# letitiabanana/PnP-OVSS

Measured on AMD Instinct MI355X. Metric: images/sec (336^2, drop_iter=4, blur+CRF), higher is better.
Workload: dtype bf16x3

## Files before the change

include/pnp_hip.h:

```cpp
#ifndef PNP_HIP_H
#define PNP_HIP_H

#include <stddef.h>
#include <stdint.h>

#ifdef __cplusplus
extern "C" {
#endif

typedef struct pnp_engine pnp_engine;

typedef struct pnp_config {
    int32_t img_size, patch, vit_dim, vit_depth, vit_heads, vit_mlp_ratio;
    float vit_ln_eps;
    int32_t txt_hidden, txt_layers, txt_heads, txt_inter;
    float txt_ln_eps;
    int32_t vocab, max_pos, enc_token_id;
    int32_t max_batch;
    int32_t max_text_len;
    int32_t stash_layer;
    int32_t compute_bf16;
    int32_t device;
} pnp_config;

// ... 226 lines not shown
enum { PNP_GEMM_G64 = 0, PNP_GEMM_G128 = 1, PNP_GEMM_G256 = 2, PNP_GEMM_WIDE = 3, PNP_GEMM_X3_WIDE = 4, PNP_GEMM_SMALL_X3 = 5 };
typedef struct pnp_gemm_plan {
    int32_t status;
    int32_t family;
    int32_t variant;
    int32_t dtype_bf16;
    int32_t n_pad;
    int32_t grid, block, smem;
    int32_t keeps_stamps;
    int32_t profiled;
    int32_t sk_full, sk_upw;
} pnp_gemm_plan;
int pnp_op_gemm_plan(int32_t form, int32_t M, int32_t N, int32_t K, int32_t lda, int32_t ldb, int32_t mode, int32_t has,
                     int32_t row_div, int32_t col_div, int32_t col_pad, int32_t n_cu, int32_t streamk_mode, int32_t sk_wgs,
                     pnp_gemm_plan* plan);
int pnp_op_vit_attention(int32_t bf16, const void* d_qk, int32_t ld_qk, int32_t D, const void* d_vt, int32_t ld_vt,
                         int32_t n_pad, void* d_ctx, int32_t B, int32_t heads, int32_t N, float scale, void* stream);
int pnp_op_vit_attention_x3(const void* d_qkv_hi, const void* d_qkv_lo, int32_t ld_qkv, int32_t D, void* d_ctx_hi, void* d_ctx_lo,
                            int32_t B, int32_t heads, int32_t N, float scale, void* stream);
int pnp_op_layernorm(const float* d_x, const float* d_w, const float* d_b, float eps, int32_t rows, int32_t D,
                     float* d_y, void* stream);
int pnp_op_xattn(int32_t bf16, int32_t mode, const void* d_nat, int32_t ld_nat, const void* d_tr, int32_t ld_tr,
                 int32_t n_pad, const void* d_x, int32_t ldx, void* d_out, int32_t ldo, float* d_probs, int32_t n_stride,
                 int32_t B, int32_t L, int32_t N, int32_t heads, void* stream);
int pnp_dbg_gemm_stamps(uint64_t* host_out, int32_t max_blocks);
int pnp_op_cast(int32_t to_bf16, const float* d_in, void* d_out, int64_t n, void* stream);
int pnp_op_sort_pairs(uint64_t* d_keys_in, uint64_t* d_keys_out, uint32_t* d_vals_in, uint32_t* d_vals_out, int64_t n,
                      int32_t begin_bit, int32_t end_bit, const size_t* h_seg_off, int32_t n_seg, void* stream);
int pnp_op_scan_i32(const int32_t* d_in, int32_t* d_out, int64_t n, int32_t inclusive, void* stream);
int pnp_op_text_self_attn(int32_t bf16, const void* d_qkv, const int64_t* d_mask, int32_t ld_mask, void* d_ctx, float* d_probs,
// ... 21 lines not shown
```

pnp-ovss_amd/csrc/kernels.h:

```cpp
#pragma once
#include <hip/hip_runtime.h>
#include <stdint.h>
#include <stddef.h>
#include "gemm.h"

namespace pnp {

struct PostDesc {
    int H, W, K, C, has_bg, pix0;
    int Kp;
    int G, Kg;
    size_t off;
    size_t qoff;
    size_t voff[2];
};

struct alignas(16) CrfEntry {
    uint32_t pixel;
    float w;
    float nr;
    uint32_t pad;
};

struct alignas(16) CrfNbr8 {
// ... 53 lines not shown

int gradcam_gather(const float* P, const float* dP, const int64_t* mask, int ld_mask, float* out, int B, int nheads,
                   int head, int L, int Nst, int PP, hipStream_t s);
int drop_step(const float* G, float* g0, float* agg, uint8_t* dropped, int32_t* picks, int iter, int B, int T, int PP,
              int npick, int max_picks, hipStream_t s);
int merge_tokens(const float* src, const int32_t* cls_off, const int32_t* tok_idx, const int32_t* cls_div,
                 const int32_t* img_cls_off, float* out, int B, int T, int PP, int Cmax, hipStream_t s);
int threshold_maps(const float* merged, const int32_t* img_cls_off, float* out, float threshold, int B, int PP, int Cmax,
                   hipStream_t s);
int upsample_maps(const float* src, const PostDesc* desc, float* maps, int B, int P, int Cmax, int maxHW, hipStream_t s);
int minmax_normalize(float* maps, const PostDesc* desc, float* stats, int B, int Kmax, int maxHW, int class_channels_only,
                     hipStream_t s);
int background_channel(float* maps, const PostDesc* desc, int B, int maxHW, hipStream_t s);
int blur_maps(const float* in, float* tmp, float* out, const PostDesc* desc, const double* wts, const int32_t* wt_off,
              int B, int Kmax, int maxH, int maxW, int max_radius, hipStream_t s);
int preprocess_images(const uint8_t* rgb, const void* desc, int B, int S, int max_H, const int32_t* coef, uint8_t* tmp,
                      const float* mean3, const float* std3, float* out, hipStream_t s);
int unary_from_maps(const float* maps, const PostDesc* desc, float* unary, int B, int maxHW, int max_kp, int group, hipStream_t s);
int argmax_remap(const float* q, const PostDesc* desc, const int32_t* lut, int lut_stride, uint8_t* labels,
                 const size_t* label_off, int pixel_major, int group, int B, int maxHW, hipStream_t s);
int confusion_hist(const uint8_t* labels, const float* gt, const PostDesc* desc, const size_t* label_off,
                   unsigned long long* hist, int n_class, int B, int maxHW, hipStream_t s);

struct JpegImage {
    int64_t data_off;
    int64_t coef_off[3];
    int64_t plane_off[3];
    int64_t rgb_off;
    int32_t data_len, H, W, ncomp, hmax, vmax, mcux, mcuy;
    int32_t h[3], v[3], tq[3], td[3], ta[3], bx[3], by[3];
// ... 74 lines not shown
```

pnp-ovss_amd/csrc/ops.hip:

```cpp
#include <cstring>

#include "engine.h"

using namespace pnp;

extern "C" int pnp_itc_similarity(const float* d_img_feat, const float* d_txt_feat, int32_t B, int32_t T, int32_t E, float* d_sim,
                                  void* stream) {
    if (!d_img_feat || !d_txt_feat || !d_sim || B <= 0 || T <= 0 || E <= 0 || E % 4) return PNP_ERR_ARG;
    return itc_similarity(d_img_feat, d_txt_feat, d_sim, B, T, E, (hipStream_t)stream);
}

static GemmArgs gemm_op_args(const void* A, const void* A_lo, int lda, const void* B, const void* B_lo, int ldb, int M, int N, int K,
                             const float* bias, int bias_on_rows, const float* resid, int ldr, float* out_f32, int ldo, void* out_t,
                             void* out_lo, int ldo_t, int mode, float* aux, int ld_aux, int row_div, int col_div, int col_pad) {
    GemmArgs g = G_(A, lda, B, ldb, M, N, K);
    g.A_lo = A_lo; g.B_lo = B_lo;
    g.bias = bias; g.bias_on_rows = bias_on_rows; g.resid = resid; g.ldr = ldr;
    g.out_f32 = out_f32; g.ldo = ldo; g.out_t = out_t; g.out_lo = out_lo; g.ldo_t = ldo_t;
    g.mode = mode; g.aux = aux; g.ld_aux = ld_aux; g.row_div = row_div; g.col_div = col_div; g.col_pad = col_pad;
    return g;
}

extern "C" int pnp_op_gemm_ex(int32_t bf, const void* d_A, int32_t lda, const void* d_B, int32_t ldb, int32_t M, int32_t N,
                              int32_t K, const float* d_bias, const float* d_resid, int32_t ldr, float* d_out_f32, int32_t ldo,
// ... 86 lines not shown
extern "C" int pnp_op_gemm_plan(int32_t form, int32_t M, int32_t N, int32_t K, int32_t lda, int32_t ldb, int32_t mode, int32_t has,
                                int32_t row_div, int32_t col_div, int32_t col_pad, int32_t n_cu, int32_t streamk_mode, int32_t sk_wgs,
                                pnp_gemm_plan* plan) {
    if (!plan || form < PNP_GEMM_FORM_F32 || form > PNP_GEMM_FORM_X3A) return PNP_ERR_ARG;
    static float there[4];
    auto p = [&](int bit) { return (has & bit) ? there : nullptr; };
    const bool x3 = form == PNP_GEMM_FORM_X3, x3a = form == PNP_GEMM_FORM_X3A;
    GemmArgs g = gemm_op_args(there, x3 ? there : nullptr, lda, there, x3 || x3a ? there : nullptr, ldb, M, N, K, p(PNP_GEMM_HAS_BIAS),
                              (has & PNP_GEMM_HAS_BIAS_ON_ROWS) ? 1 : 0, p(PNP_GEMM_HAS_RESID), 0, p(PNP_GEMM_HAS_OUT_F32), 0, p(PNP_GEMM_HAS_OUT_T),
                              p(PNP_GEMM_HAS_OUT_LO), 0, mode, p(PNP_GEMM_HAS_AUX), 0, row_div, col_div, col_pad);
    g.a_f32 = x3a;
    *plan = gemm_plan(form == PNP_GEMM_FORM_BF16 || x3, g, n_cu, streamk_mode, sk_wgs);
    return plan->status;
}

extern "C" int pnp_op_vit_attention(int32_t bf, const void* d_qk, int32_t ld_qk, int32_t D, const void* d_vt, int32_t ld_vt,
                                    int32_t n_pad, void* d_ctx, int32_t B, int32_t heads, int32_t N, float scale, void* stream) {
    if (!d_qk || !d_vt || !d_ctx || B <= 0 || heads <= 0 || N <= 0) return PNP_ERR_ARG;
    return vit_attention(bf, d_qk, ld_qk, D, d_vt, ld_vt, n_pad, d_ctx, B, heads, N, scale, (hipStream_t)stream);
}

extern "C" int pnp_op_vit_attention_x3(const void* d_qkv_hi, const void* d_qkv_lo, int32_t ld_qkv, int32_t D, void* d_ctx_hi,
                                       void* d_ctx_lo, int32_t B, int32_t heads, int32_t N, float scale, void* stream) {
    if (B <= 0 || heads <= 0 || N <= 0 || ld_qkv < 3 * D) return PNP_ERR_ARG;
    return vit_attention_x3(d_qkv_hi, d_qkv_lo, ld_qkv, D, d_ctx_hi, d_ctx_lo, B, heads, N, scale, (hipStream_t)stream);
}

extern "C" int pnp_op_layernorm(const float* d_x, const float* d_w, const float* d_b, float eps, int32_t rows, int32_t D,
                                float* d_y, void* stream) {
    return layernorm(0, d_x, d_w, d_b, eps, rows, D, d_y, nullptr, nullptr, nullptr, (hipStream_t)stream);
// ... 118 lines not shown
```

pnp-ovss_amd/csrc/pipeline_kernels.hip:

```cpp
#include "common.h"
#include "kernels.h"
#include "../../include/pnp_math.h"

namespace pnp {

__global__ void gradcam_gather_kernel(const float* __restrict__ P, const float* __restrict__ dP,
                                      const int64_t* __restrict__ mask, int ld_mask, float* __restrict__ out, int B,
                                      int nheads, int head, int L, int Nst, int PP) {
    const int idx = blockIdx.x * blockDim.x + threadIdx.x;
    const int T = L - 1;
    if (idx >= B * T * PP) return;
    const int p = idx % PP, t = (idx / PP) % T, b = idx / (PP * T);
    const size_t o = (((size_t)b * nheads + head) * L + (t + 1)) * Nst + 1 + p;
    const float g = P[o] * fmaxf(dP[o], 0.f) * (float)mask[(size_t)b * ld_mask + t + 1];
    out[idx] = g < 0.f ? 0.f : g;
}

__device__ __forceinline__ uint64_t sal_key(float v, int idx) {
    uint32_t u = __float_as_uint(v);
    u = (v != v) ? 0xffffffffu : ((u & 0x80000000u) ? ~u : (u | 0x80000000u));
    return ((uint64_t)u << 32) | (uint32_t)idx;
}

__global__ __launch_bounds__(256) void drop_accumulate_kernel(const float* __restrict__ G, float* __restrict__ g0,
// ... 129 lines not shown
    i1 = f + (f < in_size - 1 ? 1 : 0);
    w1 = lam;
    w0 = __fsub_rn(1.f, lam);
}

__global__ void upsample_kernel(const float* __restrict__ src, const PostDesc* __restrict__ desc, float* __restrict__ maps,
                                int P, int Cmax) {
    const int b = blockIdx.z, c = blockIdx.y;
    const PostDesc d = desc[b];
    if (c >= d.C) return;
    const int H = d.H, W = d.W;
    const float sh = H > 1 ? __fdiv_rn((float)(P - 1), (float)(H - 1)) : 0.f;
    const float sw = W > 1 ? __fdiv_rn((float)(P - 1), (float)(W - 1)) : 0.f;
    const float* s = src + ((size_t)b * Cmax + c) * P * P;
    float* o = maps + d.off + (size_t)(c + d.has_bg) * H * W;
    for (int i = blockIdx.x * blockDim.x + threadIdx.x; i < H * W; i += gridDim.x * blockDim.x) {
        const int y = i / W, x = i - y * W;
        int h0, h1, w0i, w1i;
        float a, bb, cc, dd;
        src_index(y, P, sh, h0, h1, a, bb);
        src_index(x, P, sw, w0i, w1i, cc, dd);
        const float v00 = s[h0 * P + w0i], v01 = s[h0 * P + w1i], v10 = s[h1 * P + w0i], v11 = s[h1 * P + w1i];
        const float top = fmaf(v00, cc, __fmul_rn(v01, dd));
        const float bot = fmaf(v10, cc, __fmul_rn(v11, dd));
        o[i] = fmaf(top, a, __fmul_rn(bot, bb));
    }
}

__global__ __launch_bounds__(256) void minmax_kernel(const float* __restrict__ maps, const PostDesc* __restrict__ desc,
                                                     float* __restrict__ stats, int Kmax, int first_k_is_class) {
    const int b = blockIdx.y, k = blockIdx.x, tid = threadIdx.x;
    const PostDesc d = desc[b];
    const int kk = first_k_is_class ? k + d.has_bg : k;
    if (kk >= d.K) return;
    if (first_k_is_class && d.C == 1) return;
    __shared__ float smn[4], smx[4];
    const float* m = maps + d.off + (size_t)kk * d.H * d.W;
    float mn = INFINITY, mx = -INFINITY;
    bool nan = false;
    const int n = d.H * d.W;
// ... 220 lines not shown
                    float* o = dst + (size_t)(y0 + rr) * W + x0 + cg * 8;
                    if (x0 + cg * 8 + 7 < W && ((reinterpret_cast<uintptr_t>(o) & 15) == 0)) {
                        reinterpret_cast<f32x4*>(o)[0] = f32x4{(float)acc[0], (float)acc[1], (float)acc[2], (float)acc[3]};
                        reinterpret_cast<f32x4*>(o)[1] = f32x4{(float)acc[4], (float)acc[5], (float)acc[6], (float)acc[7]};
                    } else {
#pragma unroll
                        for (int i = 0; i < 8; i++)
                            if (x0 + cg * 8 + i < W) o[i] = (float)acc[i];
                    }
                }
            }
        }
    }
}

struct PreImage {
    int64_t src_off, tmp_off;
    int32_t H, W, kx_off, kx_size, ky_off, ky_size;
};
__device__ __forceinline__ int clip8_fixed(int acc) {
    const int v = (acc + (1 << 21)) >> 22;
    return v < 0 ? 0 : (v > 255 ? 255 : v);
}
__global__ __launch_bounds__(256) void pre_resize_h_kernel(const uint8_t* __restrict__ rgb, const PreImage* __restrict__ desc,
                                                           int S, const int32_t* __restrict__ coef, uint8_t* __restrict__ tmp) {
    const PreImage d = desc[blockIdx.z];
    const int xo = blockIdx.x * 64 + (threadIdx.x & 63), y = blockIdx.y * 4 + (threadIdx.x >> 6);
    if (xo >= S || y >= d.H) return;
    const int32_t* t = coef + d.kx_off + (size_t)xo * (2 + d.kx_size);
    const int x0 = t[0], n = t[1];
// ... 31 lines not shown
    o[0] = __fdiv_rn(__fsub_rn(__fdiv_rn((float)clip8_fixed(a0), 255.0f), m0), s0);
    o[(size_t)S * S] = __fdiv_rn(__fsub_rn(__fdiv_rn((float)clip8_fixed(a1), 255.0f), m1), s1);
    o[(size_t)2 * S * S] = __fdiv_rn(__fsub_rn(__fdiv_rn((float)clip8_fixed(a2), 255.0f), m2), s2);
}

int preprocess_images(const uint8_t* rgb, const void* desc, int B, int S, int max_H, const int32_t* coef, uint8_t* tmp,
                      const float* mean3, const float* std3, float* out, hipStream_t s) {
    if (B <= 0 || S <= 0 || max_H <= 0) return PNP_ERR_ARG;
    const PreImage* d = reinterpret_cast<const PreImage*>(desc);
    hipLaunchKernelGGL(pre_resize_h_kernel, dim3((S + 63) / 64, (max_H + 3) / 4, B), dim3(256), 0, s, rgb, d, S, coef, tmp);
    hipLaunchKernelGGL(pre_resize_v_kernel, dim3((S + 63) / 64, (S + 3) / 4, B), dim3(256), 0, s, tmp, d, S, coef, mean3[0],
                       mean3[1], mean3[2], std3[0], std3[1], std3[2], out);
    return hipGetLastError() == hipSuccess ? PNP_OK : PNP_ERR_HIP;
}

__global__ __launch_bounds__(256) void unary_kernel(const float* __restrict__ maps, const PostDesc* __restrict__ desc,
                                                    float* __restrict__ unary, int group) {
    extern __shared__ __attribute__((aligned(16))) float utile[];
    const int b = blockIdx.y;
    const PostDesc d = desc[b];
    const int n = d.H * d.W, K = d.K, ldt = K + 1, R4 = d.Kp >> 2;
    const int f0 = group * d.Kg, f1 = f0 + K;
    const int c_lo = f0 >> 2, c_hi = group == d.G - 1 ? R4 : (f1 + 3) >> 2, nc = c_hi - c_lo;
    const float* m = maps + d.off;
    f32x4* u4 = reinterpret_cast<f32x4*>(unary + d.qoff);
    const int tid = threadIdx.x;
    for (int p0 = blockIdx.x * 256; p0 < n; p0 += gridDim.x * 256) {
        const int np = (n - p0) < 256 ? (n - p0) : 256;
        if (tid < np) {
            const int i = p0 + tid;
            const float* mi = m + i;
            float mx = mi[0];
            int k = 1;
            for (; k + 8 <= K; k += 8) {
                float v[8];
#pragma unroll
                for (int u = 0; u < 8; u++) v[u] = mi[(size_t)(k + u) * n];
#pragma unroll
                for (int u = 0; u < 8; u++)
                    if (v[u] > mx || v[u] != v[u]) mx = v[u];
            }
            for (; k < K; k++) {
                const float v = mi[(size_t)k * n];
                if (v > mx || v != v) mx = v;
            }
            float s = 0.f;
            float* row = utile + tid * ldt;
            for (k = 0; k + 8 <= K; k += 8) {
                float v[8];
#pragma unroll
                for (int u = 0; u < 8; u++) v[u] = mi[(size_t)(k + u) * n];
#pragma unroll
                for (int u = 0; u < 8; u++) {
                    const float e = pnp_expf(__fsub_rn(v[u], mx));
                    row[k + u] = e;
                    s = __fadd_rn(s, e);
                }
            }
            for (; k < K; k++) {
                const float e = pnp_expf(__fsub_rn(mi[(size_t)k * n], mx));
                row[k] = e;
                s = __fadd_rn(s, e);
            }
            for (int k = 0; k < K; k++) {
                float p = __fdiv_rn(row[k], s);
                if (p < 1e-5f) p = 1e-5f;
                else if (p > 1.0f) p = 1.0f;
                row[k] = -pnp_logf(p);
            }
        }
        __syncthreads();
        for (int item = tid; item < np * nc; item += 256) {
            const int pl = item / nc, c = c_lo + (item - pl * nc);
            const float* r = utile + pl * ldt;
            f32x4* dst = u4 + (size_t)(p0 + pl) * R4 + c;
            f32x4 v = {0.f, 0.f, 0.f, 0.f};
            if (4 * c < f0) v = *dst;
#pragma unroll
            for (int j = 0; j < 4; j++) {
                const int f = 4 * c + j;
                if (f >= f0) v[j] = f < f1 ? r[f - f0] : 0.f;
            }
            *dst = v;
        }
        __syncthreads();
    }
}

__global__ __launch_bounds__(256) void unary_wide_kernel(const float* __restrict__ maps, const PostDesc* __restrict__ desc,
                                                         float* __restrict__ unary, int group) {
    __shared__ float tiles[4][64][33];
    const int b = blockIdx.y;
    const int n = desc[b].H * desc[b].W, K = desc[b].K, R4 = desc[b].Kp >> 2, G = desc[b].G;
    const int f0 = group * desc[b].Kg, f1 = f0 + K;
    const int c_lo = f0 >> 2, c_hi = group == G - 1 ? R4 : (f1 + 3) >> 2;
    const float* m = maps + desc[b].off;
// ... 152 lines not shown

int merge_tokens(const float* src, const int32_t* cls_off, const int32_t* tok_idx, const int32_t* cls_div,
                 const int32_t* img_cls_off, float* out, int B, int T, int PP, int Cmax, hipStream_t s) {
    hipLaunchKernelGGL(merge_tokens_kernel, dim3(Cmax, B), dim3(256), 0, s, src, cls_off, tok_idx, cls_div, img_cls_off,
                       out, T, PP, Cmax);
    return ok();
}

int threshold_maps(const float* merged, const int32_t* img_cls_off, float* out, float threshold, int B, int PP, int Cmax,
                   hipStream_t s) {
    hipLaunchKernelGGL(threshold_kernel, dim3(Cmax, B), dim3(256), 0, s, merged, img_cls_off, out, threshold, PP, Cmax);
    return ok();
}

int upsample_maps(const float* src, const PostDesc* desc, float* maps, int B, int P, int Cmax, int maxHW, hipStream_t s) {
    const int nb = (maxHW + 255) / 256 < 64 ? (maxHW + 255) / 256 : 64;
    hipLaunchKernelGGL(upsample_kernel, dim3(nb, Cmax, B), dim3(256), 0, s, src, desc, maps, P, Cmax);
    return ok();
}

int minmax_normalize(float* maps, const PostDesc* desc, float* stats, int B, int Kmax, int maxHW, int class_channels_only,
                     hipStream_t s) {
    hipLaunchKernelGGL(minmax_kernel, dim3(Kmax, B), dim3(256), 0, s, maps, desc, stats, Kmax, class_channels_only);
    const int nb = (maxHW + 255) / 256 < 64 ? (maxHW + 255) / 256 : 64;
    hipLaunchKernelGGL(normalize_kernel, dim3(nb, Kmax, B), dim3(256), 0, s, maps, desc, stats, Kmax, class_channels_only);
    return ok();
}

int background_channel(float* maps, const PostDesc* desc, int B, int maxHW, hipStream_t s) {
    const int nb = (maxHW + 255) / 256 < 128 ? (maxHW + 255) / 256 : 128;
    hipLaunchKernelGGL(background_kernel, dim3(nb, B), dim3(256), 0, s, maps, desc);
    return ok();
}

int blur_maps(const float* in, float* tmp, float* out, const PostDesc* desc, const double* wts, const int32_t* wt_off,
              int B, int Kmax, int maxH, int maxW, int max_radius, hipStream_t s) {
    auto lds_for = [&](int n, size_t& l0, size_t& l1) {
        l0 = (size_t)(max_radius + 4) * sizeof(double) + (size_t)(32 * n + 2 * max_radius) * 64 * sizeof(float);
        l1 = (size_t)(max_radius + 4) * sizeof(double) + (size_t)32 * ((64 * n + 2 * max_radius) | 1) * sizeof(float);
    };
    size_t lds0, lds1;
    lds_for(1, lds0, lds1);
    int nt = lds0 > 80 * 1024 ? 4 : 1;
    lds_for(nt, lds0, lds1);
    while (nt > 1 && (lds0 > 120 * 1024 || lds1 > 120 * 1024)) lds_for(--nt, lds0, lds1);
    if (lds0 > 160 * 1024 || lds1 > 160 * 1024) return PNP_ERR_ARG;
    int nt0 = nt, nt1 = nt;
    while (nt0 > 1 && 32 * (nt0 - 1) >= maxH) nt0--;
    while (nt1 > 1 && 64 * (nt1 - 1) >= maxW) nt1--;
    lds_for(nt0, lds0, lds1);
    size_t d0, d1;
    lds_for(nt1, d0, d1);
    lds1 = d1;
    static std::atomic<uint32_t> opted0{0}, opted1{0};
    if (lds_opt_in(opted0, reinterpret_cast<const void*>(blur_axis_kernel<0>), 160 * 1024) != PNP_OK) return PNP_ERR_HIP;
    if (lds_opt_in(opted1, reinterpret_cast<const void*>(blur_axis_kernel<1>), 160 * 1024) != PNP_OK) return PNP_ERR_HIP;
    const int tiles0 = ((maxW + 63) / 64) * ((maxH + 32 * nt0 - 1) / (32 * nt0));
    const int tiles1 = ((maxW + 64 * nt1 - 1) / (64 * nt1)) * ((maxH + 31) / 32);
    hipLaunchKernelGGL(blur_axis_kernel<0>, dim3(tiles0, Kmax, B), dim3(256 * nt0), lds0, s, in, tmp, desc, wts, wt_off, max_radius, nt0);
    hipLaunchKernelGGL(blur_axis_kernel<1>, dim3(tiles1, Kmax, B), dim3(256 * nt1), lds1, s, tmp, out, desc, wts, wt_off, max_radius, nt1);
    return ok();
}

int unary_from_maps(const float* maps, const PostDesc* desc, float* unary, int B, int maxHW, int max_kp, int group, hipStream_t s) {
    const int nb = (maxHW + 255) / 256 < 256 ? (maxHW + 255) / 256 : 256;
    const size_t smem = (size_t)256 * (max_kp + 1) * sizeof(float);
    static std::atomic<uint32_t> opted{0};
    if (lds_opt_in(opted, reinterpret_cast<const void*>(unary_kernel), 160 * 1024) != PNP_OK) return PNP_ERR_HIP;
    if (max_kp >= 32) {
        const int nbw = (maxHW + 255) / 256 < 2048 ? (maxHW + 255) / 256 : 2048;
        hipLaunchKernelGGL(unary_wide_kernel, dim3(nbw, B), dim3(256), 0, s, maps, desc, unary, group);
        return ok();
    }
    hipLaunchKernelGGL(unary_kernel, dim3(nb, B), dim3(256), smem, s, maps, desc, unary, group);
    return ok();
}

int argmax_remap(const float* q, const PostDesc* desc, const int32_t* lut, int lut_stride, uint8_t* labels,
                 const size_t* label_off, int pixel_major, int group, int B, int maxHW, hipStream_t s) {
    const int nb = (maxHW + 255) / 256 < 256 ? (maxHW + 255) / 256 : 256;
    hipLaunchKernelGGL(argmax_kernel, dim3(nb, B), dim3(256), 0, s, q, desc, lut, lut_stride, labels, label_off, pixel_major, group);
    return ok();
}
// ... 11 lines not shown
```

pnp-ovss_amd/pnp_ovss/hip.py:

```python
import ctypes as C
import os

import numpy as np
import torch

_HERE = os.path.dirname(os.path.abspath(__file__))
LIB_PATH = os.environ.get("PNP_HIP_LIB") or os.path.join(_HERE, "libpnp_hip.so")


class PnpConfig(C.Structure):
    _fields_ = [(n, C.c_int32) for n in ("img_size", "patch", "vit_dim", "vit_depth", "vit_heads", "vit_mlp_ratio")] + \
               [("vit_ln_eps", C.c_float)] + \
               [(n, C.c_int32) for n in ("txt_hidden", "txt_layers", "txt_heads", "txt_inter")] + \
               [("txt_ln_eps", C.c_float)] + \
               [(n, C.c_int32) for n in ("vocab", "max_pos", "enc_token_id", "max_batch", "max_text_len",
                                         "stash_layer", "compute_bf16", "device")]


class PnpPostBatch(C.Structure):
    _fields_ = [("B", C.c_int32),
                ("H", C.POINTER(C.c_int32)), ("W", C.POINTER(C.c_int32)),
                ("n_classes", C.POINTER(C.c_int32)), ("has_bg", C.POINTER(C.c_int32)),
                ("img_cls_off", C.POINTER(C.c_int32)), ("cls_off", C.POINTER(C.c_int32)),
                ("tok_idx", C.POINTER(C.c_int32)), ("cls_div", C.POINTER(C.c_int32)),
# ... 8 lines not shown
                ("d_rgb", C.c_void_p), ("d_unary", C.c_void_p)]


class PnpCrfTerm(C.Structure):
    _fields_ = [("dims", C.c_int32), ("d_features", C.c_void_p)]


class PnpCrfLatticeView(C.Structure):
    _fields_ = [("D1", C.c_int32), ("images", C.c_int32), ("cap", C.c_int64), ("points", C.c_int64), ("entries", C.c_int64)] + \
               [(n, C.c_void_p) for n in ("bary", "offset", "vals", "ent", "seg_lo", "seg_hi", "idbase", "n1", "n2", "nbr8", "norm")]


class PnpGemmPlan(C.Structure):
    _fields_ = [(n, C.c_int32) for n in ("status", "family", "variant", "dtype_bf16", "n_pad", "grid", "block", "smem",
                                         "keeps_stamps", "profiled", "sk_full", "sk_upw")]


_lib = None


def load_library():
    global _lib
    if _lib is not None:
        return _lib
    if not os.path.exists(LIB_PATH):
        raise RuntimeError(f"{LIB_PATH} not built: run `python -c 'import __graft_entry__ as g; g.build()'` "
                           f"or `make -C pnp-ovss_amd/csrc` (there is no CPU fallback)")
    lib = C.CDLL(LIB_PATH)
    vp, i32, i64, f32 = C.c_void_p, C.c_int32, C.c_int64, C.c_float
    sig = {
# ... 26 lines not shown
        "pnp_blur_minmax": (i32, [vp, vp]),
        "pnp_densecrf": (i32, [vp, i32, f32, f32, f32, f32, f32, vp]),
        "pnp_remap_hist": (i32, [vp, i32, vp, vp, i32, vp]),
        "pnp_postprocess": (i32, [vp, vp, i32, f32, i32, i32, vp, vp, i32, vp]),
        "pnp_postprocess_pair": (i32, [vp, vp, vp, i32, f32, i32, vp, vp, vp, vp, i32, vp]),
        "pnp_get_buffer": (i32, [vp, C.c_char_p, C.POINTER(vp), C.POINTER(C.c_size_t)]),
        "pnp_profile_enable": (i32, [vp, i32]),
        "pnp_profile_read": (i32, [vp, C.POINTER(i64), C.POINTER(C.c_double), C.POINTER(C.c_double)]),
        "pnp_profile_read_stage": (i32, [vp, i32, C.POINTER(i64), C.POINTER(C.c_double), C.POINTER(C.c_double)]),
        "pnp_op_gemm": (i32, [i32, vp, i32, vp, i32, i32, i32, i32, vp, vp, i32, vp, i32, i32, vp]),
        "pnp_op_gemm_ex": (i32, [i32, vp, i32, vp, i32, i32, i32, i32, vp, vp, i32, vp, i32, vp, i32, i32, vp]),
        "pnp_op_gemm_tokcols": (i32, [i32, vp, i32, vp, i32, i32, i32, i32, vp, vp, i32, i32, i32, vp]),
        "pnp_op_gemm_args": (i32, [i32, vp, i32, vp, i32, i32, i32, i32, vp, i32, vp, i32, vp, i32, vp, i32, i32, vp, i32, i32, i32,
                                   i32, vp]),
        "pnp_op_gemm_plan": (i32, [i32] * 14 + [C.POINTER(PnpGemmPlan)]),
        "pnp_op_vit_attention": (i32, [i32, vp, i32, i32, vp, i32, i32, vp, i32, i32, i32, f32, vp]),
        "pnp_op_vit_attention_x3": (i32, [vp, vp, i32, i32, vp, vp, i32, i32, i32, f32, vp]),
        "pnp_preprocess_images": (i32, [vp, vp, i32, i32, i32, vp, vp, C.POINTER(C.c_float), C.POINTER(C.c_float), vp, vp]),
        "pnp_op_layernorm": (i32, [vp, vp, vp, f32, i32, i32, vp, vp]),
        "pnp_op_cast": (i32, [i32, vp, vp, i64, vp]),
        "pnp_jpeg_decode": (i32, [vp, vp, vp, vp, i32, i32, vp, vp, vp, i64, vp, vp, i32, i32, vp, vp]),
        "pnp_overlay_labels": (i32, [vp, vp, vp, i32, vp, C.c_double, vp, vp]),
        "pnp_jpeg_encode": (i32, [vp, vp, i32, vp, vp, vp, vp, vp, i64, C.POINTER(i64), vp]),
        "pnp_op_split": (i32, [vp, vp, vp, i64, vp]),
        "pnp_op_gemm_x3": (i32, [vp, vp, i32, vp, vp, i32, i32, i32, i32, vp, i32, vp, i32, vp, i32, vp, vp, i32, i32, i32, i32, vp]),
        "pnp_op_gemm_x3a": (i32, [vp, i32, vp, vp, i32, i32, i32, i32, vp, vp, i32, vp, i32, i32, vp, i32, vp]),
        "pnp_dbg_gemm_stamps": (i32, [vp, i32]),
        "pnp_op_xattn": (i32, [i32, i32, vp, i32, vp, i32, i32, vp, i32, vp, i32, vp, i32, i32, i32, i32, i32, vp]),
        "pnp_op_sort_pairs": (i32, [vp, vp, vp, vp, i64, i32, i32, vp, i32, vp]),
        "pnp_op_scan_i32": (i32, [vp, vp, i64, i32, vp]),
# ... 39 lines not shown
    _lib = lib
    return lib


EXPORTED = ["pnp_create", "pnp_create_shared", "pnp_destroy", "pnp_last_error", "pnp_workspace_bytes", "pnp_load_weight",
            "pnp_finalize_weights", "pnp_vit_forward", "pnp_text_forward_xattn", "pnp_xattn_grad",
            "pnp_gradcam_gather", "pnp_compute_gradcam", "pnp_drop_step", "pnp_drop_loop", "pnp_post_reserve",
            "pnp_post_prepare", "pnp_merge_tokens", "pnp_threshold_upsample", "pnp_blur_minmax", "pnp_densecrf",
            "pnp_remap_hist", "pnp_postprocess", "pnp_postprocess_pair", "pnp_get_buffer", "pnp_profile_enable", "pnp_profile_read", "pnp_op_gemm", "pnp_op_gemm_ex", "pnp_op_layernorm", "pnp_op_cast", "pnp_op_xattn", "pnp_dbg_gemm_stamps", "pnp_op_gemm_tokcols", "pnp_op_vit_attention", "pnp_preprocess_images",
            "pnp_cross_kv", "pnp_profile_read_stage", "pnp_op_split", "pnp_op_gemm_x3", "pnp_op_gemm_x3a",
            "pnp_xattn_grad_layer", "pnp_compute_gradcam_layer", "pnp_drop_loop_layer", "pnp_allocated_bytes",
            "pnp_op_vit_attention_x3", "pnp_jpeg_decode", "pnp_op_sort_pairs", "pnp_op_scan_i32", "pnp_set_tuning",
            "pnp_streamk_status", "pnp_text_forward_text", "pnp_project_normalize", "pnp_itc_similarity",
            "pnp_op_text_self_attn", "pnp_op_text_self_attn_bwd", "pnp_op_layernorm_ex", "pnp_op_layernorm_bwd",
            "pnp_op_text_embed", "pnp_op_itm_head", "pnp_op_itm_grad_seed", "pnp_op_patchify", "pnp_op_cls_rows",
            "pnp_op_gemm_args", "pnp_op_gemm_plan", "pnp_overlay_labels", "pnp_jpeg_encode",
            "pnp_crf_create", "pnp_crf_destroy", "pnp_crf_allocated_bytes", "pnp_crf_last_error", "pnp_crf_set_batch",
            "pnp_crf_infer", "pnp_crf_set_batch_aniso", "pnp_crf_set_compat", "pnp_crf_start", "pnp_crf_step", "pnp_crf_read",
            "pnp_crf_kl", "pnp_crf_create_terms", "pnp_crf_set_batch_terms", "pnp_crf_set_term_compat", "pnp_crf_infer_terms",
            "pnp_crf_step_terms", "pnp_crf_lattice_points", "pnp_crf_reserve_grad", "pnp_crf_infer_terms_saved",
            "pnp_crf_backward_terms", "pnp_crf_lattice_view_get", "pnp_crf_probe_filter"]


PROJ_NAMES = ("vision_proj.weight", "vision_proj.bias", "text_proj.weight", "text_proj.bias")


class _DevView:

    def __init__(self, ptr, shape, typestr):
        self.__cuda_array_interface__ = {"shape": tuple(shape), "typestr": typestr, "data": (int(ptr), False),
                                         "version": 2, "strides": None}
# ... 566 lines not shown
    return n.value, t.value


GEMM_FORMS = ("f32", "bf16", "x3", "x3a")
GEMM_FAMILIES = ("g64", "g128", "g256", "wide", "x3_wide", "small_x3")
GEMM_HAS = {"bias": 1, "bias_on_rows": 2, "resid": 4, "out_f32": 8, "out_t": 16, "out_lo": 32, "aux": 64}


def gemm_plan(form, M, N, K, has=(), mode=0, row_div=0, col_div=0, col_pad=0, n_cu=256, streamk=1, sk_wgs=None, lda=None, ldb=None):
    plan = PnpGemmPlan()
    bits = sum(GEMM_HAS[h] for h in has)
    load_library().pnp_op_gemm_plan(GEMM_FORMS.index(form), M, N, K, K if lda is None else lda, K if ldb is None else ldb, mode, bits,
                                    row_div, col_div, col_pad, n_cu, streamk, n_cu if sk_wgs is None else sk_wgs, C.byref(plan))
    plan.name = GEMM_FAMILIES[plan.family] if plan.status == 0 else None
    return plan
```

Measured before the change: 221.1.

## Add full-line strip blur kernels, vectorize upsample, stage unary maps via LDS

Adds a strip-based separable blur kernel that loads whole lines of the map into LDS with reflected halos and computes eight outputs per task, chosen by a new blur planner when the strip fits under an LDS cap; otherwise the old tiled kernels are used. The upsample kernel now writes four outputs per thread with vector stores, and the unary softmax kernel stages the class maps into a column-major LDS tile with coalesced vector loads instead of strided global reads per pixel. These aim to cut uncoalesced global traffic and redundant halo loads in postprocessing, at the cost of more LDS per block and extra code paths.

```diff
diff --git a/include/pnp_hip.h b/include/pnp_hip.h
--- a/include/pnp_hip.h
+++ b/include/pnp_hip.h
@@ -264,6 +264,12 @@
 int pnp_op_gemm_plan(int32_t form, int32_t M, int32_t N, int32_t K, int32_t lda, int32_t ldb, int32_t mode, int32_t has,
                      int32_t row_div, int32_t col_div, int32_t col_pad, int32_t n_cu, int32_t streamk_mode, int32_t sk_wgs,
                      pnp_gemm_plan* plan);
+enum { PNP_BLUR_STRIP_LDS_MAX = 80 * 1024 };
+typedef struct pnp_blur_plan {
+    int32_t status;
+    int32_t strip[2], lines[2], nt[2], grid[2], block[2], smem[2];
+} pnp_blur_plan;
+int pnp_op_blur_plan(int32_t H, int32_t W, int32_t radius, pnp_blur_plan* plan);
 int pnp_op_vit_attention(int32_t bf16, const void* d_qk, int32_t ld_qk, int32_t D, const void* d_vt, int32_t ld_vt,
                          int32_t n_pad, void* d_ctx, int32_t B, int32_t heads, int32_t N, float scale, void* stream);
 int pnp_op_vit_attention_x3(const void* d_qkv_hi, const void* d_qkv_lo, int32_t ld_qkv, int32_t D, void* d_ctx_hi, void* d_ctx_lo,
diff --git a/pnp-ovss_amd/csrc/kernels.h b/pnp-ovss_amd/csrc/kernels.h
--- a/pnp-ovss_amd/csrc/kernels.h
+++ b/pnp-ovss_amd/csrc/kernels.h
@@ -91,6 +91,8 @@
 int background_channel(float* maps, const PostDesc* desc, int B, int maxHW, hipStream_t s);
 int blur_maps(const float* in, float* tmp, float* out, const PostDesc* desc, const double* wts, const int32_t* wt_off,
               int B, int Kmax, int maxH, int maxW, int max_radius, hipStream_t s);
+typedef pnp_blur_plan BlurPlan;
+BlurPlan blur_plan(int maxH, int maxW, int max_radius);
 int preprocess_images(const uint8_t* rgb, const void* desc, int B, int S, int max_H, const int32_t* coef, uint8_t* tmp,
                       const float* mean3, const float* std3, float* out, hipStream_t s);
 int unary_from_maps(const float* maps, const PostDesc* desc, float* unary, int B, int maxHW, int max_kp, int group, hipStream_t s);
diff --git a/pnp-ovss_amd/csrc/ops.hip b/pnp-ovss_amd/csrc/ops.hip
--- a/pnp-ovss_amd/csrc/ops.hip
+++ b/pnp-ovss_amd/csrc/ops.hip
@@ -124,6 +124,12 @@
     return plan->status;
 }
 
+extern "C" int pnp_op_blur_plan(int32_t H, int32_t W, int32_t radius, pnp_blur_plan* plan) {
+    if (!plan) return PNP_ERR_ARG;
+    *plan = blur_plan(H, W, radius);
+    return plan->status;
+}
+
 extern "C" int pnp_op_vit_attention(int32_t bf, const void* d_qk, int32_t ld_qk, int32_t D, const void* d_vt, int32_t ld_vt,
                                     int32_t n_pad, void* d_ctx, int32_t B, int32_t heads, int32_t N, float scale, void* stream) {
     if (!d_qk || !d_vt || !d_ctx || B <= 0 || heads <= 0 || N <= 0) return PNP_ERR_ARG;
diff --git a/pnp-ovss_amd/csrc/pipeline_kernels.hip b/pnp-ovss_amd/csrc/pipeline_kernels.hip
--- a/pnp-ovss_amd/csrc/pipeline_kernels.hip
+++ b/pnp-ovss_amd/csrc/pipeline_kernels.hip
@@ -167,16 +167,35 @@
     const float sw = W > 1 ? __fdiv_rn((float)(P - 1), (float)(W - 1)) : 0.f;
     const float* s = src + ((size_t)b * Cmax + c) * P * P;
     float* o = maps + d.off + (size_t)(c + d.has_bg) * H * W;
-    for (int i = blockIdx.x * blockDim.x + threadIdx.x; i < H * W; i += gridDim.x * blockDim.x) {
-        const int y = i / W, x = i - y * W;
-        int h0, h1, w0i, w1i;
-        float a, bb, cc, dd;
+    const int qpr = (W + 3) >> 2;
+    const bool vec = (W & 3) == 0 && (reinterpret_cast<uintptr_t>(o) & 15) == 0;
+    for (int i = blockIdx.x * blockDim.x + threadIdx.x; i < H * qpr; i += gridDim.x * blockDim.x) {
+        const int y = i / qpr, x0 = (i - y * qpr) * 4;
+        int h0, h1;
+        float a, bb;
         src_index(y, P, sh, h0, h1, a, bb);
-        src_index(x, P, sw, w0i, w1i, cc, dd);
-        const float v00 = s[h0 * P + w0i], v01 = s[h0 * P + w1i], v10 = s[h1 * P + w0i], v11 = s[h1 * P + w1i];
-        const float top = fmaf(v00, cc, __fmul_rn(v01, dd));
-        const float bot = fmaf(v10, cc, __fmul_rn(v11, dd));
-        o[i] = fmaf(top, a, __fmul_rn(bot, bb));
+        const float* s0 = s + h0 * P;
+        const float* s1 = s + h1 * P;
+        float r[4];
+#pragma unroll
+        for (int j = 0; j < 4; j++) {
+            const int x = x0 + j < W ? x0 + j : W - 1;
+            int w0i, w1i;
+            float cc, dd;
+            src_index(x, P, sw, w0i, w1i, cc, dd);
+            const float v00 = s0[w0i], v01 = s0[w1i], v10 = s1[w0i], v11 = s1[w1i];
+            const float top = fmaf(v00, cc, __fmul_rn(v01, dd));
+            const float bot = fmaf(v10, cc, __fmul_rn(v11, dd));
+            r[j] = fmaf(top, a, __fmul_rn(bot, bb));
+        }
+        float* dst = o + (size_t)y * W + x0;
+        if (vec) {
+            *reinterpret_cast<f32x4*>(dst) = f32x4{r[0], r[1], r[2], r[3]};
+        } else {
+#pragma unroll
+            for (int j = 0; j < 4; j++)
+                if (x0 + j < W) dst[j] = r[j];
+        }
     }
 }
 
@@ -427,6 +446,108 @@
     }
 }
 
+constexpr int BLUR_STRIP = 32;
+template <int AXIS, int LINES>
+__global__ __launch_bounds__(512) void blur_strip_kernel(const float* __restrict__ in, float* __restrict__ out,
+                                                        const PostDesc* __restrict__ desc, const double* __restrict__ wts,
+                                                        const int32_t* __restrict__ wt_off, int max_radius) {
+    constexpr int SW = LINES;
+    extern __shared__ __attribute__((aligned(16))) double tile[];
+    double* wl = tile;
+    float* xs = reinterpret_cast<float*>(tile + ((max_radius + 3) & ~1));
+    const int b = blockIdx.z, k = blockIdx.y;
+    const PostDesc d = desc[b];
+    if (k >= d.K) return;
+    const int H = d.H, W = d.W;
+    const int n = AXIS == 0 ? H : W, m = AXIS == 0 ? W : H;
+    const int s0 = blockIdx.x * SW;
+    if (s0 >= m) return;
+    const int sv = m - s0 < SW ? m - s0 : SW;
+    const double* w = wts + wt_off[b];
+    const int radius = wt_off[b + 1] - wt_off[b] - 1;
+    const float* src = in + d.off + (size_t)k * H * W;
+    float* dst = out + d.off + (size_t)k * H * W;
+    const int tid = threadIdx.x, nthr = blockDim.x;
+    for (int j = tid; j <= radius; j += nthr) wl[j] = w[j];
+    const int n8 = (n + 7) & ~7, ext = n8 + 2 * radius;
+    const int ld = AXIS == 0 ? SW : (ext | 1);
+    auto at = [&](int l, int e) { return AXIS == 0 ? e * ld + l : l * ld + e; };
+    if ((W & 3) == 0 && (reinterpret_cast<uintptr_t>(src) & 15) == 0) {
+        const int ppr = AXIS == 0 ? sv >> 2 : W >> 2;
+        const int total = (AXIS == 0 ? H : sv) * ppr;
+        for (int i0 = tid; i0 < total; i0 += 8 * nthr) {
+            f32x4 v[8];
+            int r[8], p[8];
+#pragma unroll
+            for (int u = 0; u < 8; u++) {
+                const int i = i0 + u * nthr;
+                r[u] = i / ppr;
+                p[u] = (i - r[u] * ppr) * 4;
+                const size_t g = AXIS == 0 ? (size_t)r[u] * W + s0 + p[u] : (size_t)(s0 + r[u]) * W + p[u];
+                v[u] = i < total ? *reinterpret_cast<const f32x4*>(src + g) : f32x4{0.f, 0.f, 0.f, 0.f};
+            }
+#pragma unroll
+            for (int u = 0; u < 8; u++) {
+                if (i0 + u * nthr < total) {
+                    if constexpr (AXIS == 0) {
+                        *reinterpret_cast<f32x4*>(xs + (radius + r[u]) * ld + p[u]) = v[u];
+                    } else {
+#pragma unroll
+                        for (int j = 0; j < 4; j++) xs[r[u] * ld + radius + p[u] + j] = v[u][j];
+                    }
+                }
+            }
+        }
+    } else {
+        const int rl = AXIS == 0 ? sv : W;
+        const int total = (AXIS == 0 ? H : sv) * rl;
+        constexpr int NF = 16;
+        for (int i0 = tid; i0 < total; i0 += NF * nthr) {
+            float v[NF];
+            int r[NF], c[NF];
+#pragma unroll
+            for (int u = 0; u < NF; u++) {
+                const int i = i0 + u * nthr;
+                r[u] = i / rl;
+                c[u] = i - r[u] * rl;
+                const size_t g = AXIS == 0 ? (size_t)r[u] * W + s0 + c[u] : (size_t)(s0 + r[u]) * W + c[u];
+                v[u] = i < total ? src[g] : 0.f;
+            }
+#pragma unroll
+            for (int u = 0; u < NF; u++)
+                if (i0 + u * nthr < total) xs[AXIS == 0 ? at(c[u], radius + r[u]) : at(r[u], radius + c[u])] = v[u];
+        }
+    }
+    __syncthreads();
+    for (int i = tid; i < (ext - n) * sv; i += nthr) {
+        const int a = i / sv, l = i - a * sv;
+        const int e = a < radius ? a : a + n;
+        xs[at(l, e)] = xs[at(l, radius + reflect_fast(e - radius, n))];
+    }
+    __syncthreads();
+    const int tasks = (n8 >> 3) * sv;
+    for (int task = tid; task < tasks; task += nthr) {
+        const int g = task / sv, l = task - g * sv;
+        double acc[8];
+        blur_window8(xs + at(l, radius + g * 8), AXIS == 0 ? ld : 1, wl, radius, acc);
+        if constexpr (AXIS == 0) {
+#pragma unroll
+            for (int i = 0; i < 8; i++)
+                if (g * 8 + i < H) dst[(size_t)(g * 8 + i) * W + s0 + l] = (float)acc[i];
+        } else {
+            float* o = dst + (size_t)(s0 + l) * W + g * 8;
+            if (g * 8 + 7 < W && ((reinterpret_cast<uintptr_t>(o) & 15) == 0)) {
+                reinterpret_cast<f32x4*>(o)[0] = f32x4{(float)acc[0], (float)acc[1], (float)acc[2], (float)acc[3]};
+                reinterpret_cast<f32x4*>(o)[1] = f32x4{(float)acc[4], (float)acc[5], (float)acc[6], (float)acc[7]};
+            } else {
+#pragma unroll
+                for (int i = 0; i < 8; i++)
+                    if (g * 8 + i < W) o[i] = (float)acc[i];
+            }
+        }
+    }
+}
+
 struct PreImage {
     int64_t src_off, tmp_off;
     int32_t H, W, kx_off, kx_size, ky_off, ky_size;
@@ -488,72 +609,87 @@
     return hipGetLastError() == hipSuccess ? PNP_OK : PNP_ERR_HIP;
 }
 
+constexpr int UNARY_LDP = 260;
 __global__ __launch_bounds__(256) void unary_kernel(const float* __restrict__ maps, const PostDesc* __restrict__ desc,
                                                     float* __restrict__ unary, int group) {
     extern __shared__ __attribute__((aligned(16))) float utile[];
+    constexpr int LDP = UNARY_LDP;
     const int b = blockIdx.y;
     const PostDesc d = desc[b];
-    const int n = d.H * d.W, K = d.K, ldt = K + 1, R4 = d.Kp >> 2;
+    const int n = d.H * d.W, K = d.K, R4 = d.Kp >> 2;
     const int f0 = group * d.Kg, f1 = f0 + K;
     const int c_lo = f0 >> 2, c_hi = group == d.G - 1 ? R4 : (f1 + 3) >> 2, nc = c_hi - c_lo;
     const float* m = maps + d.off;
     f32x4* u4 = reinterpret_cast<f32x4*>(unary + d.qoff);
     const int tid = threadIdx.x;
+    const bool vec = (n & 3) == 0 && (reinterpret_cast<uintptr_t>(m) & 15) == 0;
     for (int p0 = blockIdx.x * 256; p0 < n; p0 += gridDim.x * 256) {
         const int np = (n - p0) < 256 ? (n - p0) : 256;
+        if (vec) {
+            const int q = np >> 2, total = K * q;
+            for (int i0 = tid; i0 < total; i0 += 8 * 256) {
+                f32x4 v[8];
+                int at[8];
+#pragma unroll
+                for (int u = 0; u < 8; u++) {
+                    const int i = i0 + u * 256;
+                    const int k = i / q, px = (i - k * q) * 4;
+                    at[u] = k * LDP + px;
+                    v[u] = i < total ? *reinterpret_cast<const f32x4*>(m + (size_t)k * n + p0 + px) : f32x4{0.f, 0.f, 0.f, 0.f};
+                }
+#pragma unroll
+                for (int u = 0; u < 8; u++)
+                    if (i0 + u * 256 < total) *reinterpret_cast<f32x4*>(utile + at[u]) = v[u];
+            }
+        } else {
+            const int total = K * np;
+            for (int i0 = tid; i0 < total; i0 += 8 * 256) {
+                float v[8];
+                int at[8];
+#pragma unroll
+                for (int u = 0; u < 8; u++) {
+                    const int i = i0 + u * 256;
+                    const int k = i / np, px = i - k * np;
+                    at[u] = k * LDP + px;
+                    v[u] = i < total ? m[(size_t)k * n + p0 + px] : 0.f;
+                }
+#pragma unroll
+                for (int u = 0; u < 8; u++)
+                    if (i0 + u * 256 < total) utile[at[u]] = v[u];
+            }
+        }
+        __syncthreads();
         if (tid < np) {
-            const int i = p0 + tid;
-            const float* mi = m + i;
-            float mx = mi[0];
-            int k = 1;
-            for (; k + 8 <= K; k += 8) {
-                float v[8];
-#pragma unroll
-                for (int u = 0; u < 8; u++) v[u] = mi[(size_t)(k + u) * n];
-#pragma unroll
-                for (int u = 0; u < 8; u++)
-                    if (v[u] > mx || v[u] != v[u]) mx = v[u];
-            }
-            for (; k < K; k++) {
-                const float v = mi[(size_t)k * n];
+            float* col = utile + tid;
+            float mx = col[0];
+            for (int k = 1; k < K; k++) {
+                const float v = col[k * LDP];
                 if (v > mx || v != v) mx = v;
             }
             float s = 0.f;
-            float* row = utile + tid * ldt;
-            for (k = 0; k + 8 <= K; k += 8) {
-                float v[8];
-#pragma unroll
-                for (int u = 0; u < 8; u++) v[u] = mi[(size_t)(k + u) * n];
-#pragma unroll
-                for (int u = 0; u < 8; u++) {
-                    const float e = pnp_expf(__fsub_rn(v[u], mx));
-                    row[k + u] = e;
-                    s = __fadd_rn(s, e);
-                }
-            }
-            for (; k < K; k++) {
-                const float e = pnp_expf(__fsub_rn(mi[(size_t)k * n], mx));
-                row[k] = e;
+            for (int k = 0; k < K; k++) {
+                const float e = pnp_expf(__fsub_rn(col[k * LDP], mx));
+                col[k * LDP] = e;
                 s = __fadd_rn(s, e);
             }
             for (int k = 0; k < K; k++) {
-                float p = __fdiv_rn(row[k], s);
+                float p = __fdiv_rn(col[k * LDP], s);
                 if (p < 1e-5f) p = 1e-5f;
                 else if (p > 1.0f) p = 1.0f;
-                row[k] = -pnp_logf(p);
+                col[k * LDP] = -pnp_logf(p);
             }
         }
         __syncthreads();
         for (int item = tid; item < np * nc; item += 256) {
             const int pl = item / nc, c = c_lo + (item - pl * nc);
-            const float* r = utile + pl * ldt;
+            const float* r = utile + pl;
             f32x4* dst = u4 + (size_t)(p0 + pl) * R4 + c;
             f32x4 v = {0.f, 0.f, 0.f, 0.f};
             if (4 * c < f0) v = *dst;
 #pragma unroll
             for (int j = 0; j < 4; j++) {
                 const int f = 4 * c + j;
-                if (f >= f0) v[j] = f < f1 ? r[f - f0] : 0.f;
+                if (f >= f0) v[j] = f < f1 ? r[(f - f0) * LDP] : 0.f;
             }
             *dst = v;
         }
@@ -736,7 +872,8 @@
 }
 
 int upsample_maps(const float* src, const PostDesc* desc, float* maps, int B, int P, int Cmax, int maxHW, hipStream_t s) {
-    const int nb = (maxHW + 255) / 256 < 64 ? (maxHW + 255) / 256 : 64;
+    const int items = maxHW / 4 + 256;
+    const int nb = (items + 255) / 256 < 64 ? (items + 255) / 256 : 64;
     hipLaunchKernelGGL(upsample_kernel, dim3(nb, Cmax, B), dim3(256), 0, s, src, desc, maps, P, Cmax);
     return ok();
 }
@@ -755,40 +892,85 @@
     return ok();
 }
 
-int blur_maps(const float* in, float* tmp, float* out, const PostDesc* desc, const double* wts, const int32_t* wt_off,
-              int B, int Kmax, int maxH, int maxW, int max_radius, hipStream_t s) {
+BlurPlan blur_plan(int maxH, int maxW, int max_radius) {
+    BlurPlan p{};
+    if (maxH <= 0 || maxW <= 0 || max_radius < 0) { p.status = PNP_ERR_ARG; return p; }
+    const size_t taps = (size_t)(max_radius + 4) * sizeof(double);
     auto lds_for = [&](int n, size_t& l0, size_t& l1) {
-        l0 = (size_t)(max_radius + 4) * sizeof(double) + (size_t)(32 * n + 2 * max_radius) * 64 * sizeof(float);
-        l1 = (size_t)(max_radius + 4) * sizeof(double) + (size_t)32 * ((64 * n + 2 * max_radius) | 1) * sizeof(float);
+        l0 = taps + (size_t)(32 * n + 2 * max_radius) * 64 * sizeof(float);
+        l1 = taps + (size_t)32 * ((64 * n + 2 * max_radius) | 1) * sizeof(float);
     };
     size_t lds0, lds1;
     lds_for(1, lds0, lds1);
     int nt = lds0 > 80 * 1024 ? 4 : 1;
     lds_for(nt, lds0, lds1);
     while (nt > 1 && (lds0 > 120 * 1024 || lds1 > 120 * 1024)) lds_for(--nt, lds0, lds1);
-    if (lds0 > 160 * 1024 || lds1 > 160 * 1024) return PNP_ERR_ARG;
-    int nt0 = nt, nt1 = nt;
-    while (nt0 > 1 && 32 * (nt0 - 1) >= maxH) nt0--;
-    while (nt1 > 1 && 64 * (nt1 - 1) >= maxW) nt1--;
-    lds_for(nt0, lds0, lds1);
-    size_t d0, d1;
-    lds_for(nt1, d0, d1);
-    lds1 = d1;
-    static std::atomic<uint32_t> opted0{0}, opted1{0};
-    if (lds_opt_in(opted0, reinterpret_cast<const void*>(blur_axis_kernel<0>), 160 * 1024) != PNP_OK) return PNP_ERR_HIP;
-    if (lds_opt_in(opted1, reinterpret_cast<const void*>(blur_axis_kernel<1>), 160 * 1024) != PNP_OK) return PNP_ERR_HIP;
-    const int tiles0 = ((maxW + 63) / 64) * ((maxH + 32 * nt0 - 1) / (32 * nt0));
-    const int tiles1 = ((maxW + 64 * nt1 - 1) / (64 * nt1)) * ((maxH + 31) / 32);
-    hipLaunchKernelGGL(blur_axis_kernel<0>, dim3(tiles0, Kmax, B), dim3(256 * nt0), lds0, s, in, tmp, desc, wts, wt_off, max_radius, nt0);
-    hipLaunchKernelGGL(blur_axis_kernel<1>, dim3(tiles1, Kmax, B), dim3(256 * nt1), lds1, s, tmp, out, desc, wts, wt_off, max_radius, nt1);
+    const bool tiles_fit = lds0 <= 160 * 1024 && lds1 <= 160 * 1024;
+    int ntp[2] = {nt, nt};
+    while (ntp[0] > 1 && 32 * (ntp[0] - 1) >= maxH) ntp[0]--;
+    while (ntp[1] > 1 && 64 * (ntp[1] - 1) >= maxW) ntp[1]--;
+    for (int a = 0; a < 2; a++) {
+        const int n = a == 0 ? maxH : maxW, m = a == 0 ? maxW : maxH;
+        const int n8 = (n + 7) & ~7, ext = n8 + 2 * max_radius;
+        const size_t per_line = (size_t)(a == 0 ? ext : (ext | 1)) * sizeof(float);
+        if (taps + BLUR_STRIP * per_line <= (size_t)PNP_BLUR_STRIP_LDS_MAX) {
+            long best_slots = -1;
+            for (int lines = BLUR_STRIP; lines >= 24; lines -= 8) {
+                const int strips = (m + lines - 1) / lines, tasks = (n8 >> 3) * lines;
+                for (int t = 256; t <= 512; t += 64) {
+                    const long slots = (long)strips * ((tasks + t - 1) / t) * t;
+                    if (best_slots < 0 || slots < best_slots) {
+                        best_slots = slots;
+                        p.lines[a] = lines;
+                        p.grid[a] = strips;
+                        p.block[a] = t;
+                    }
+                }
+            }
+            p.strip[a] = 1;
+            p.smem[a] = (int32_t)(taps + p.lines[a] * per_line);
+        } else {
+            if (!tiles_fit) { p = BlurPlan{}; p.status = PNP_ERR_ARG; return p; }
+            size_t l0, l1;
+            lds_for(ntp[a], l0, l1);
+            p.nt[a] = ntp[a];
+            p.grid[a] = a == 0 ? ((maxW + 63) / 64) * ((maxH + 32 * ntp[0] - 1) / (32 * ntp[0]))
+                               : ((maxW + 64 * ntp[1] - 1) / (64 * ntp[1])) * ((maxH + 31) / 32);
+            p.block[a] = 256 * ntp[a];
+            p.smem[a] = (int32_t)(a == 0 ? l0 : l1);
+        }
+    }
+    return p;
+}
+
+int blur_maps(const float* in, float* tmp, float* out, const PostDesc* desc, const double* wts, const int32_t* wt_off,
+              int B, int Kmax, int maxH, int maxW, int max_radius, hipStream_t s) {
+    const BlurPlan p = blur_plan(maxH, maxW, max_radius);
+    if (p.status != PNP_OK) return p.status;
+    using StripFn = void (*)(const float*, float*, const PostDesc*, const double*, const int32_t*, int);
+    static const StripFn strips[2][2] = {{blur_strip_kernel<0, 32>, blur_strip_kernel<1, 32>}, {blur_strip_kernel<0, 24>, blur_strip_kernel<1, 24>}};
+    static std::atomic<uint32_t> opted[3][2];
+    const float* src[2] = {in, tmp};
+    float* dst[2] = {tmp, out};
+    for (int a = 0; a < 2; a++) {
+        const dim3 grid(p.grid[a], Kmax, B), block(p.block[a]);
+        const int form = !p.strip[a] ? 0 : p.lines[a] == BLUR_STRIP ? 1 : 2;
+        const void* fn = form ? reinterpret_cast<const void*>(strips[form - 1][a])
+                              : a == 0 ? reinterpret_cast<const void*>(blur_axis_kernel<0>) : reinterpret_cast<const void*>(blur_axis_kernel<1>);
+        if (lds_opt_in(opted[form][a], fn, 160 * 1024) != PNP_OK) return PNP_ERR_HIP;
+        if (form) {
+            hipLaunchKernelGGL(strips[form - 1][a], grid, block, p.smem[a], s, src[a], dst[a], desc, wts, wt_off, max_radius);
+        } else {
+            if (a == 0) hipLaunchKernelGGL(blur_axis_kernel<0>, grid, block, p.smem[a], s, src[a], dst[a], desc, wts, wt_off, max_radius, p.nt[a]);
+            else hipLaunchKernelGGL(blur_axis_kernel<1>, grid, block, p.smem[a], s, src[a], dst[a], desc, wts, wt_off, max_radius, p.nt[a]);
+        }
+    }
     return ok();
 }
 
 int unary_from_maps(const float* maps, const PostDesc* desc, float* unary, int B, int maxHW, int max_kp, int group, hipStream_t s) {
     const int nb = (maxHW + 255) / 256 < 256 ? (maxHW + 255) / 256 : 256;
-    const size_t smem = (size_t)256 * (max_kp + 1) * sizeof(float);
-    static std::atomic<uint32_t> opted{0};
-    if (lds_opt_in(opted, reinterpret_cast<const void*>(unary_kernel), 160 * 1024) != PNP_OK) return PNP_ERR_HIP;
+    const size_t smem = (size_t)max_kp * UNARY_LDP * sizeof(float);
     if (max_kp >= 32) {
         const int nbw = (maxHW + 255) / 256 < 2048 ? (maxHW + 255) / 256 : 2048;
         hipLaunchKernelGGL(unary_wide_kernel, dim3(nbw, B), dim3(256), 0, s, maps, desc, unary, group);
diff --git a/pnp-ovss_amd/pnp_ovss/hip.py b/pnp-ovss_amd/pnp_ovss/hip.py
--- a/pnp-ovss_amd/pnp_ovss/hip.py
+++ b/pnp-ovss_amd/pnp_ovss/hip.py
@@ -46,6 +46,10 @@
 class PnpGemmPlan(C.Structure):
     _fields_ = [(n, C.c_int32) for n in ("status", "family", "variant", "dtype_bf16", "n_pad", "grid", "block", "smem",
                                          "keeps_stamps", "profiled", "sk_full", "sk_upw")]
+
+
+class PnpBlurPlan(C.Structure):
+    _fields_ = [("status", C.c_int32)] + [(n, C.c_int32 * 2) for n in ("strip", "lines", "nt", "grid", "block", "smem")]
 
 
 _lib = None
@@ -102,6 +106,7 @@
         "pnp_op_gemm_args": (i32, [i32, vp, i32, vp, i32, i32, i32, i32, vp, i32, vp, i32, vp, i32, vp, i32, i32, vp, i32, i32, i32,
                                    i32, vp]),
         "pnp_op_gemm_plan": (i32, [i32] * 14 + [C.POINTER(PnpGemmPlan)]),
+        "pnp_op_blur_plan": (i32, [i32, i32, i32, C.POINTER(PnpBlurPlan)]),
         "pnp_op_vit_attention": (i32, [i32, vp, i32, i32, vp, i32, i32, vp, i32, i32, i32, f32, vp]),
         "pnp_op_vit_attention_x3": (i32, [vp, vp, i32, i32, vp, vp, i32, i32, i32, f32, vp]),
         "pnp_preprocess_images": (i32, [vp, vp, i32, i32, i32, vp, vp, C.POINTER(C.c_float), C.POINTER(C.c_float), vp, vp]),
@@ -171,7 +176,7 @@
             "pnp_streamk_status", "pnp_text_forward_text", "pnp_project_normalize", "pnp_itc_similarity",
             "pnp_op_text_self_attn", "pnp_op_text_self_attn_bwd", "pnp_op_layernorm_ex", "pnp_op_layernorm_bwd",
             "pnp_op_text_embed", "pnp_op_itm_head", "pnp_op_itm_grad_seed", "pnp_op_patchify", "pnp_op_cls_rows",
-            "pnp_op_gemm_args", "pnp_op_gemm_plan", "pnp_overlay_labels", "pnp_jpeg_encode",
+            "pnp_op_gemm_args", "pnp_op_gemm_plan", "pnp_op_blur_plan", "pnp_overlay_labels", "pnp_jpeg_encode",
             "pnp_crf_create", "pnp_crf_destroy", "pnp_crf_allocated_bytes", "pnp_crf_last_error", "pnp_crf_set_batch",
             "pnp_crf_infer", "pnp_crf_set_batch_aniso", "pnp_crf_set_compat", "pnp_crf_start", "pnp_crf_step", "pnp_crf_read",
             "pnp_crf_kl", "pnp_crf_create_terms", "pnp_crf_set_batch_terms", "pnp_crf_set_term_compat", "pnp_crf_infer_terms",
@@ -768,3 +773,12 @@
                                     row_div, col_div, col_pad, n_cu, streamk, n_cu if sk_wgs is None else sk_wgs, C.byref(plan))
     plan.name = GEMM_FAMILIES[plan.family] if plan.status == 0 else None
     return plan
+
+
+BLUR_STRIP_LDS_MAX = 80 * 1024
+
+
+def blur_plan(H, W, radius):
+    plan = PnpBlurPlan()
+    load_library().pnp_op_blur_plan(H, W, radius, C.byref(plan))
+    return plan
```

Result: no change. 222.9 (median of 6 runs) (+0.8%).
